# lunarlab-gatech/SLIDE_SLAM

Hardware: AMD Instinct MI355X
Metric: pose-graph updates/sec + ms/Gauss-Newton iter, 8-robot 10k-landmark graph (higher is better)
Workload: dtype f64

## Files before the change

### slide_slam_amd/csrc/solver_kernels.hip

```cpp
#include <hip/hip_runtime.h>
#include <algorithm>
#include <cstring>

#include "graph_dev.hpp"
#include "kernels.hpp"
#include "sl_math.hpp"

namespace sl {

struct BufPtrs { double* p[8]; };

__device__ inline void pose_retract12(const double* in12, const double* d6, int chart, double* out12) {
  to12(retract(from12(in12), d6, chart), out12);
}
__device__ inline void lm_retract(int type, const double* in, const double* d, int chart, double* out) {
  if (type == VT_POINT) {
    out[0] = in[0] + d[0]; out[1] = in[1] + d[1]; out[2] = in[2] + d[2];
  } else if (type == VT_CUBE) {
    pose_retract12(in, d, chart, out);
    out[12] = in[12] + d[6]; out[13] = in[13] + d[7]; out[14] = in[14] + d[8];
  } else {
    out[3] = in[3] + d[0]; out[4] = in[4] + d[1]; out[5] = in[5] + d[2];
    out[0] = in[0] + d[3]; out[1] = in[1] + d[4]; out[2] = in[2] + d[5];
    out[6] = in[6] + d[6];
// ... 928 lines not shown
void launch_gather_args(void* stage, const void* segs, int nseg, hipStream_t s) {
  GatherArgs A{};
  std::memcpy(A.seg, segs, (size_t)nseg * sizeof(ScatterSeg));
  if (nseg > 0) hipLaunchKernelGGL(k_gather_args, dim3(nseg, 4), dim3(256), 0, s, static_cast<unsigned char*>(stage), A);
}
void launch_gather(void* stage, unsigned desc_off, int nseg, hipStream_t s) {
  if (nseg > 0) hipLaunchKernelGGL(k_gather, dim3(nseg, 4), dim3(256), 0, s, static_cast<unsigned char*>(stage), desc_off);
}
void launch_scatter(const void* stage, unsigned desc_off, int nseg, hipStream_t s) {
  if (nseg > 0) hipLaunchKernelGGL(k_scatter, dim3(nseg, 8), dim3(256), 0, s, static_cast<const unsigned char*>(stage), desc_off);
}

__device__ __forceinline__ void k_pad_rhs_body(const GraphDev& G, int bid) {
  const int n = 6 * G.P, NT = G.T * NB;
  const long long t = (long long)bid * 256 + threadIdx.x;
  if (t < NT) {
    const int c = (int)t;
    G.S[(size_t)c * G.ld + NT + (size_t)G.nbr * NB] = c < G.col0 ? G.yv[c] : ((c < n) ? -G.pose_g[c] : 0.0);
    return;
  }
  const long long u = t - NT;
  const int npad = NT - n;
  if (u >= (long long)npad * NT) return;
  const int r = n + (int)(u / NT), c = (int)(u % NT);
  if (c > r || c < G.col0) return;
  if (G.first && c < G.first[G.T - 1] * NB) return;
  G.S[(size_t)c * G.ld + r] = (c == r) ? 1.0 : 0.0;
  if (G.save_S0) G.S0[(size_t)c * G.ld + r] = (c == r) ? 1.0 : 0.0;
}
__global__ __launch_bounds__(256) void k_pad_rhs(GraphDev G) { k_pad_rhs_body(G, blockIdx.x); }
__global__ __launch_bounds__(256) void k_pad_rhs_b(const GraphDev* __restrict__ Gs) {
  const GraphDev G = Gs[blockIdx.z];
  k_pad_rhs_body(G, blockIdx.x);
}

template <int MODE>
__device__ __forceinline__ void k_backsub_body(const GraphDev& G) {
  const int wave = threadIdx.x >> 6, lane = threadIdx.x & 63;
  if (MODE != 2) {
    const int t = blockIdx.x * 256 + threadIdx.x;
    if (t < 6 * G.P) G.pose_delta[t] = G.dp[t];
  }
  for (int l = blockIdx.x * 4 + wave; l < G.L; l += gridDim.x * 4) {
    const int D = lm_dim(G.lm_type[l]);
    double rhs[9];
#pragma unroll
    for (int k = 0; k < 9; ++k) rhs[k] = 0.0;
    if (MODE == 2) {
#pragma unroll
      for (int k = 0; k < 9; ++k) if (k < D) rhs[k] = G.lm_t[9 * (size_t)l + k];
    } else {
      for (int q = G.lm_ptr[l] + lane; q < G.lm_ptr[l + 1]; q += 64) {
        const int f = G.lm_fids[q];
        const double* E = G.ebuf + G.lf_eoff[f];
        const double* d = G.dp + 6 * (size_t)G.lf_pose[f];
        double dd[6];
#pragma unroll
        for (int a = 0; a < 6; ++a) dd[a] = d[a];
#pragma unroll
        for (int k = 0; k < 9; ++k) {
          if (k < D) {
            double s = 0.0;
#pragma unroll
            for (int a = 0; a < 6; ++a) s += E[a * D + k] * dd[a];
            rhs[k] += s;
          }
        }
      }
#pragma unroll
      for (int k = 0; k < 9; ++k) {
#pragma unroll
        for (int m = 32; m >= 1; m >>= 1) rhs[k] += __shfl_xor(rhs[k], m);
      }
    }
    if (MODE == 1) {
      if (lane == 0) {
#pragma unroll
        for (int k = 0; k < 9; ++k) G.lm_t[9 * (size_t)l + k] = rhs[k];
      }
      continue;
    }
#pragma unroll
    for (int k = 0; k < 9; ++k) if (k < D) rhs[k] += G.lm_g[9 * (size_t)l + k];
    if (lane < D) {
      const double* Hi = G.lm_Hinv + 81 * (size_t)l + lane * D;
      double s = 0.0;
#pragma unroll
      for (int c = 0; c < 9; ++c) if (c < D) s += Hi[c] * rhs[c];
      G.lm_delta[9 * (size_t)l + lane] = -s;
    }
  }
}
template <int MODE>
__global__ __launch_bounds__(256) void k_backsub(GraphDev G) { k_backsub_body<MODE>(G); }
template <int MODE>
__global__ __launch_bounds__(256) void k_backsub_b(const GraphDev* __restrict__ Gs) { k_backsub_body<MODE>(Gs[blockIdx.z]); }

__device__ __forceinline__ void k_shared_pack_body(const GraphDev& G, int what, double* __restrict__ buf) {
  const int w = what == 0 ? 54 : (what == 1 ? 9 : 15);
  const int t = blockIdx.x * blockDim.x + threadIdx.x;
  const int sidx = t / w, k = t - sidx * w;
  if (sidx >= G.n_slots) return;
  const int l = G.sh_lid[sidx];
  const bool live = l >= 0 && (what != 2 || G.sh_owner[sidx]);
  const double* src = what == 0 ? G.lm_Hacc + 54 * (size_t)(l < 0 ? 0 : l) : (what == 1 ? G.lm_t + 9 * (size_t)(l < 0 ? 0 : l) : G.lm_val + 15 * (size_t)(l < 0 ? 0 : l));
  buf[t] = live ? src[k] : 0.0;
}
__global__ void k_shared_pack(GraphDev G, int what, double* __restrict__ buf) { k_shared_pack_body(G, what, buf); }
__global__ void k_shared_unpack(GraphDev G, int what, const double* __restrict__ buf) {
  const int w = what == 0 ? 54 : (what == 1 ? 9 : 15);
  const int t = blockIdx.x * blockDim.x + threadIdx.x;
  const int sidx = t / w, k = t - sidx * w;
  if (sidx >= G.n_slots) return;
  const int l = G.sh_lid[sidx];
  if (l < 0) return;
  double* dst = what == 0 ? G.lm_Hacc + 54 * (size_t)l : (what == 1 ? G.lm_t + 9 * (size_t)l : G.lm_val + 15 * (size_t)l);
  const int nv = what == 2 ? (G.lm_type[l] == VT_POINT ? 3 : (G.lm_type[l] == VT_CUBE ? 15 : 7)) : w;
  if (k < nv) dst[k] = buf[t];
}

__global__ __launch_bounds__(256) void k_border_clear_b(const GraphDev* __restrict__ Gs) {
  const GraphDev G = Gs[blockIdx.z];
  if (!G.arrow || G.nbr <= 0) return;
  const long long nrow = (long long)G.nbr * NB, ncol = (long long)G.T * NB;
  const long long nb = (long long)(G.nbr + 1) * NB * G.nbr * NB;
  if (G.seg_tab) {
    const int* st = G.seg_tab;
    const int nseg = st[0], ntile = G.nbr * G.T;
    for (int tile = blockIdx.x; tile < ntile; tile += gridDim.x) {
      const int t = tile % G.nbr, c = tile / G.nbr;
      bool on = false;
      for (int q = 0; q < nseg; ++q) on = on || (st[1 + nseg + q * (G.nbr + 1) + t] <= c && c < st[1 + q]);
      if (!on) continue;
      double* base = G.S + (size_t)c * NB * G.ld + (size_t)(G.T + t) * NB;
      for (int e = threadIdx.x; e < NB * NB; e += 256) base[(size_t)(e >> 6) * G.ld + (e & 63)] = 0.0;
    }
    (void)nb;
    return;
  }
  for (long long t = (long long)blockIdx.x * 256 + threadIdx.x; t < nrow * ncol; t += (long long)gridDim.x * 256)
    G.S[(size_t)(t / nrow) * G.ld + (size_t)G.T * NB + (size_t)(t % nrow)] = 0.0;
}
__global__ __launch_bounds__(256) void k_border_fill_b(const GraphDev* __restrict__ Gs) {
  const GraphDev G = Gs[blockIdx.z];
  if (!G.arrow || G.nbr <= 0) return;
  const int sidx = blockIdx.x * 4 + (threadIdx.x >> 6), lane = threadIdx.x & 63;
  if (sidx >= G.n_slots) return;
  const int l = G.sh_lid[sidx];
  if (l < 0) return;
  const int o = G.lm_bord[l];
  if (o < 0) return;
  const int D = lm_dim(G.lm_type[l]);
  const int a = lane / D, k = lane - a * D;
  if (lane < 6 * D) {
    for (int q = G.lm_ptr[l]; q < G.lm_ptr[l + 1]; ++q) {
      const int f = G.lm_fids[q];
      const double e = G.ebuf[G.lf_eoff[f] + a * D + k];
      double* dst = G.S + (size_t)(6 * G.lf_pose[f] + a) * G.ld + (size_t)G.T * NB + o + k;
      *dst += e;
    }
  }
  const double* acc = G.lm_Hacc + 54 * (size_t)l;
  if (lane < D * (D + 1) / 2) {
    int r = 0;
    while ((r + 1) * (r + 2) / 2 <= lane) ++r;
    const int c = lane - r * (r + 1) / 2;
    G.bord0[(size_t)(o + c) * G.ldb + o + r] = acc[lane];
  }
  if (lane < D) G.bord0[(size_t)(o + lane) * G.ldb + (size_t)G.nbr * NB] = -acc[45 + lane];
}
__global__ __launch_bounds__(256) void k_sep_extract_b(const GraphDev* __restrict__ Gs, int max_sep) {
  const GraphDev G = Gs[blockIdx.z];
  if (!G.arrow || !G.pose_sep || G.nsep <= 0) return;
  __shared__ int s_q;
  if (threadIdx.x == 0) s_q = -1;
  __syncthreads();
  for (int p = threadIdx.x; p < G.P; p += 256)
    if (G.pose_sep[p] == 6 * (int)blockIdx.x) s_q = p;
  __syncthreads();
  const int q = s_q;
  if (q < 0) return;
  (void)max_sep;
  const int tid = threadIdx.x, oq = G.pose_sep[q], NT = G.T * NB;
  const size_t ld = G.ld, ldb = G.ldb;
  const size_t brow = (size_t)G.T * NB;
  const int nb_rows = G.nbr * NB;
  const int r_end = G.prof ? min(NT, (G.prof[(6 * q + 5) / NB] + 1) * NB) : NT;
  const int n_strip = r_end - 6 * q;
  const int part = blockIdx.y;
  for (int e = tid; part == 0 && e < 6 * n_strip; e += 256) {
    const int a = e / n_strip, r = 6 * q + e % n_strip, c = 6 * q + a;
    if (r < c) continue;
    double* src = G.S + (size_t)c * ld + r;
    const double v = *src;
    const int pr = r / 6;
    if (pr < G.P) {
      const int orr = G.pose_sep[pr];
      if (orr >= 0) G.bord0[(size_t)(oq + a) * ldb + orr + (r - 6 * pr)] = v;
      else G.S[(size_t)r * ld + brow + oq + a] = v;
    }
    *src = (r == c) ? 1.0 : 0.0;
  }
  for (int e = tid; part == 1 && e < 6 * nb_rows; e += 256) {
    const int a = e / nb_rows, b = e % nb_rows;
    double* src = G.S + (size_t)(6 * q + a) * ld + brow + b;
    const double v = *src;
    double* dst = G.bord0 + (size_t)(oq + a) * ldb + b;
    if (v != 0.0) { *dst = v; *src = 0.0; }
    else if (b >= G.nsep * NB && *dst != 0.0) *dst = 0.0;
  }
  if (part == 0 && tid < 6) {
    double* src = G.S + (size_t)(6 * q + tid) * ld + brow + (size_t)G.nbr * NB;
    G.bord0[(size_t)(oq + tid) * ldb + (size_t)G.nbr * NB] = *src;
    *src = 0.0;
  }
  if (part == 0 && blockIdx.x == 0)
    for (int p = G.nsep_dim + tid; p < G.nsep * NB; p += 256) G.bord0[(size_t)p * ldb + p] = 1.0;
  const int c_beg = G.first ? G.first[(6 * q) / NB] * NB : 0;
  for (int e = tid; part == 2 && e < 6 * (6 * q - c_beg); e += 256) {
    const int a = e % 6, c = c_beg + e / 6, r = 6 * q + a;
    const int pc = c / 6;
    if (pc >= G.P || G.pose_sep[pc] >= 0) continue;
    double* src = G.S + (size_t)c * ld + r;
    G.S[(size_t)c * ld + brow + oq + a] = *src;
    *src = 0.0;
  }
}
__global__ __launch_bounds__(256) void k_sep_pose_scatter_b(const GraphDev* __restrict__ Gs, BufPtrs X) {
  const GraphDev G = Gs[blockIdx.z];
  if (!G.arrow || !G.pose_sep || G.nsep <= 0) return;
  const int t = blockIdx.x * 256 + threadIdx.x;
  if (t >= 6 * G.P) return;
  const int o = G.pose_sep[t / 6];
  if (o >= 0) G.dp[t] = X.p[blockIdx.z][o + t % 6];
}
__global__ __launch_bounds__(256) void k_border_fill_lam_b(const GraphDev* __restrict__ Gs) {
  const GraphDev G = Gs[blockIdx.z];
  if (!G.arrow || !G.gh_bord || G.nbr <= 0) return;
  const int t = blockIdx.x * 256 + threadIdx.x;
  const int q = t / 36, e = t - 36 * q;
  if (q >= G.n_ghost) return;
  const int o = G.gh_bord[q];
  if (o < 0) return;
  const int k = e / 6, a = e - 6 * k;
  G.S[(size_t)(6 * G.gh_pose[q] + a) * G.ld + (size_t)G.T * NB + o + k] = G.gh_J[36 * (size_t)q + 6 * k + a];
  if (G.gh_first[q] && a == 0) {
    G.bord0[(size_t)(o + k) * G.ldb + o + k] = -1.0;
    G.bord0[(size_t)(o + k) * G.ldb + (size_t)G.nbr * NB] = -G.gh_r[6 * (size_t)q + k];
  }
}
__device__ __forceinline__ size_t sep_packed_addr(int row, int col, int Ts, int hTa, int hTL) {
  const int tj = col / NB, cc = col - tj * NB, hb = hTL - hTa;
  const size_t off = (size_t)(NB * NB) * ((size_t)tj * (Ts + 1) - (size_t)tj * (tj - 1) / 2 - (size_t)hb * min(tj, hTa));
  const int height = Ts + 1 - tj - (tj < hTa ? hb : 0);
  int r = row - tj * NB;
  if (tj < hTa && row >= hTL * NB) r -= hb * NB;
  return off + (size_t)cc * ((size_t)height * NB) + (size_t)r;
}
__device__ __forceinline__ bool sep_packed_hole(int row, int col, int hTa, int hTL) { return col < hTa * NB && row >= hTa * NB && row < hTL * NB; }
__device__ __forceinline__ double* sep_slot(const SepLayout& Y, int vr, int vc, bool packed) {
  const int Tt = Y.Ts + Y.nl;
  if (packed) return Y.packed + sep_packed_addr(vr, vc, Tt, Y.hTa, Y.hTL);
  if (vc < Y.Ts * NB) return Y.sys + (size_t)vc * ((size_t)(Tt + 1) * NB) + vr;
  return Y.bord + (size_t)(vc - Y.Ts * NB) * ((size_t)(Y.nl + 1) * NB) + (vr - Y.Ts * NB);
}
struct SepGatherArgs {
  int n, packed;
  SepLayout Y;
  const double* bord[8]; int ldb[8]; int nbr[8]; const int* map[8];
  const int* tmask;
  unsigned robot_mask;
  int split_col; unsigned mask_b; double* sys2; int ld2; double* bord2;
};
constexpr int SEP_GATHER_COLS = 8;
__global__ __launch_bounds__(256) void k_sep_gather(SepGatherArgs A) {
  const SepLayout& Y = A.Y;
  const int vr = blockIdx.x * 256 + threadIdx.x;
  const int NL = Y.Ts * NB, NT = (Y.Ts + Y.nl) * NB;
  if (vr > NT) return;
  const bool rhs = vr == NT;
  const int gr = rhs ? 0 : (vr < NL ? (vr < Y.ms ? vr : -1) : (vr - NL < Y.lam ? Y.ms + vr - NL : -1));
  const unsigned rmask = A.tmask ? (rhs ? ~0u : (unsigned)A.tmask[vr / NB]) : ~0u;
  int lrow[8];
#pragma unroll
  for (int r = 0; r < 8; ++r) {
    lrow[r] = -1;
    if (r < A.n && gr >= 0 && ((rmask >> r) & 1u) && ((A.robot_mask >> r) & 1u)) lrow[r] = rhs ? A.nbr[r] * NB : A.map[r][gr];
  }
#pragma unroll 2
  for (int vc = blockIdx.y * SEP_GATHER_COLS; vc < (int)(blockIdx.y + 1) * SEP_GATHER_COLS && vc < NT; ++vc) {
    if (!rhs && vr < vc) continue;
    if (sep_packed_hole(vr, vc, Y.hTa, Y.hTL)) continue;
    const int gc = vc < NL ? (vc < Y.ms ? vc : -1) : (vc - NL < Y.lam ? Y.ms + vc - NL : -1);
    double s = 0.0, s2 = 0.0;
    if (gc < 0 || gr < 0) {
      s = (vr == vc && vc < NL) ? 1.0 : 0.0;
    } else if (vr == vc && ((vc >= Y.gap[0] && vc < Y.gap[1]) || (vc >= Y.gap[2] && vc < Y.gap[3]))) {
      s = A.packed ? 0.0 : 1.0;
    } else {
      const unsigned cand = (A.tmask ? (unsigned)A.tmask[vc / NB] & rmask : ~0u) & A.robot_mask;
      double v[8];
#pragma unroll
      for (int r = 0; r < 8; ++r) {
        v[r] = 0.0;
        if (r < A.n && ((cand >> r) & 1u) && lrow[r] >= 0) {
          const int lc = A.map[r][gc];
          const int lr = lrow[r];
          if (lc >= 0) v[r] = A.bord[r][(size_t)min(lr, lc) * A.ldb[r] + max(lr, lc)];
        }
      }
      if (A.split_col >= 0 && vc >= A.split_col) {
        double va[8], vb[8];
#pragma unroll
        for (int r = 0; r < 8; ++r) { const bool b = (A.mask_b >> r) & 1u; va[r] = b ? 0.0 : v[r]; vb[r] = b ? v[r] : 0.0; }
        s = ((va[0] + va[1]) + (va[2] + va[3])) + ((va[4] + va[5]) + (va[6] + va[7]));
        s2 = ((vb[0] + vb[1]) + (vb[2] + vb[3])) + ((vb[4] + vb[5]) + (vb[6] + vb[7]));
      } else {
        s = ((v[0] + v[1]) + (v[2] + v[3])) + ((v[4] + v[5]) + (v[6] + v[7]));
      }
    }
    *sep_slot(Y, vr, vc, A.packed != 0) = s;
    if (A.split_col >= 0 && vc >= A.split_col) {
      if (vc < NL) A.sys2[(size_t)(vc - A.split_col) * A.ld2 + (vr - A.split_col)] = s2;
      else A.bord2[(size_t)(vc - NL) * ((size_t)(Y.nl + 1) * NB) + (vr - NL)] = s2;
    }
  }
}
__global__ __launch_bounds__(256) void k_sep_unpack(SepLayout Y, int c0, int c1, int to_packed) {
  const int vr = blockIdx.x * 256 + threadIdx.x, vc = c0 * NB + blockIdx.y;
  const int NT = (Y.Ts + Y.nl) * NB;
  if (vr > NT || vc >= NT || vc >= c1 * NB || vr < vc / NB * NB) return;
  if (sep_packed_hole(vr, vc, Y.hTa, Y.hTL)) return;
  if (to_packed) { *sep_slot(Y, vr, vc, true) = *sep_slot(Y, vr, vc, false); return; }
  double v = *sep_slot(Y, vr, vc, true);
  if (vr == vc && ((vc >= Y.gap[0] && vc < Y.gap[1]) || (vc >= Y.gap[2] && vc < Y.gap[3]))) v = 1.0;
  *sep_slot(Y, vr, vc, false) = v;
}
__global__ __launch_bounds__(256) void k_lam_prepare(const double* __restrict__ bord, int nl, int lam, double* __restrict__ out) {
  const int r = blockIdx.x * 256 + threadIdx.x, c = blockIdx.y;
  const int NT = nl * NB, ld = (nl + 1) * NB;
  if (r > NT || c >= NT) return;
  const bool rhs = r == NT;
  if (!rhs && r < c) return;
  double v;
  if (c < lam && (rhs || r < lam)) v = -bord[(size_t)c * ld + r];
  else v = (r == c) ? 1.0 : 0.0;
  out[(size_t)c * ld + r] = v;
}
struct SepScatterArgs { int n, m, ms; const double* xs; const double* xl; double* xloc[8]; const int* map[8]; };
__global__ __launch_bounds__(256) void k_sep_xloc(SepScatterArgs A) {
  const int g = blockIdx.x * 256 + threadIdx.x, r = blockIdx.y;
  if (g >= A.m || r >= A.n) return;
  const int lc = A.map[r][g];
  if (lc >= 0) A.xloc[r][lc] = g < A.ms ? A.xs[g] : A.xl[g - A.ms];
}
__global__ __launch_bounds__(256) void k_sep_lm_delta_b(const GraphDev* __restrict__ Gs, SepScatterArgs A, const int* __restrict__ sep_off) {
  const GraphDev G = Gs[blockIdx.z];
  const int t = blockIdx.x * 256 + threadIdx.x;
  const int sidx = t / 9, k = t - 9 * sidx;
  if (sidx >= G.n_slots) return;
  const int l = G.sh_lid[sidx];
  if (l < 0) return;
  if (k < lm_dim(G.lm_type[l])) G.lm_delta[9 * (size_t)l + k] = A.xs[sep_off[sidx] + k];
}
__global__ void k_ghost_exchange(GraphDev G, int what, double* __restrict__ buf) {
  const int t = blockIdx.x * blockDim.x + threadIdx.x;
  if (t >= 12 * G.n_gslots) return;
  if (what == 0) {
    const int p = G.gslot_pose[t / 12];
    buf[t] = p >= 0 ? G.pose_est[12 * (size_t)p + t % 12] : 0.0;
  } else {
    G.ghost_val[t] = buf[t];
  }
}

struct GhostBufs { double* p[8]; };
__global__ void k_ghost_exchange_b(const GraphDev* __restrict__ Gs, int what, GhostBufs B) {
  const GraphDev G = Gs[blockIdx.z];
  double* buf = B.p[blockIdx.z];
  const int t = blockIdx.x * blockDim.x + threadIdx.x;
  if (t >= 12 * G.n_gslots) return;
  if (what == 0) {
    const int p = G.gslot_pose[t / 12];
    buf[t] = p >= 0 ? G.pose_est[12 * (size_t)p + t % 12] : 0.0;
  } else {
    G.ghost_val[t] = buf[t];
  }
}
__global__ void k_ghost_refresh_local(const GraphDev* __restrict__ Gs, int n) {
  const GraphDev G = Gs[blockIdx.z];
  const int t = blockIdx.x * blockDim.x + threadIdx.x;
  if (t >= 12 * G.n_gslots) return;
  double v = 0.0;
  for (int q = 0; q < n; ++q) {
    const int p = Gs[q].gslot_pose[t / 12];
    v += p >= 0 ? Gs[q].pose_est[12 * (size_t)p + t % 12] : 0.0;
  }
  G.ghost_val[t] = v;
}
void launch_ghost_refresh_local(const GraphDev* d, int n, int n_gslots, hipStream_t s) {
  if (n_gslots <= 0 || n <= 0) return;
  hipLaunchKernelGGL(k_ghost_refresh_local, dim3((12 * n_gslots + 127) / 128, 1, n), dim3(128), 0, s, d, n);
}
void launch_ghost_exchange_batched(const GraphDev* d, int n, int n_gslots, int what, double* const* bufs, hipStream_t s) {
  if (n_gslots <= 0 || n <= 0) return;
  GhostBufs B{};
  for (int i = 0; i < n; ++i) B.p[i] = bufs[i];
  hipLaunchKernelGGL(k_ghost_exchange_b, dim3((12 * n_gslots + 127) / 128, 1, n), dim3(128), 0, s, d, what, B);
}

__device__ __forceinline__ void k_estimate_body(const GraphDev& G) {
  const int t = blockIdx.x * blockDim.x + threadIdx.x;
  if (t < G.P) {
    pose_retract12(G.pose_val + 12 * (size_t)t, G.pose_delta + 6 * (size_t)t, G.chart, G.pose_est + 12 * (size_t)t);
  } else if (t < G.P + G.L) {
    const int l = t - G.P;
    lm_retract(G.lm_type[l], G.lm_val + 15 * (size_t)l, G.lm_delta + 9 * (size_t)l, G.chart, G.lm_est + 15 * (size_t)l);
  }
}
__global__ void k_estimate(GraphDev G) { k_estimate_body(G); }
__global__ void k_estimate_predict(GraphDev G, int pose, double* __restrict__ out) {
  k_estimate_body(G);
  const int t = blockIdx.x * blockDim.x + threadIdx.x;
  int dirty = 0;
  if (t < G.P) {
    double mx = 0.0;
#pragma unroll
    for (int k = 0; k < 6; ++k) mx = fmax(mx, fabs(G.pose_delta[6 * (size_t)t + k]));
    if (mx >= G.relin_thr) dirty = mark_dirty_pose(G, t);
  } else if (t < G.P + G.L) {
    const int l = t - G.P;
    const int d = lm_dim(G.lm_type[l]);
    double mx = 0.0;
    for (int k = 0; k < d; ++k) mx = fmax(mx, fabs(G.lm_delta[9 * (size_t)l + k]));
    if (mx >= G.relin_thr) dirty = mark_dirty_lm(G, l);
  }
  if (__ballot(dirty > 0)) {
#pragma unroll
    for (int off = 32; off > 0; off >>= 1) dirty = max(dirty, __shfl_xor(dirty, off));
    if ((threadIdx.x & 63) == 0 && dirty > 0) atomicMax(&G.status[5], dirty);
  }
  if (out) {
    __shared__ int s_last;
    __threadfence();
    __syncthreads();
    if (threadIdx.x == 0) {
      int* cnt = reinterpret_cast<int*>(out + 16);
      const int a = atomicAdd(cnt, 1);
      s_last = (a == (int)gridDim.x - 1) ? 1 : 0;
      if (s_last) *cnt = 0;
    }
    __syncthreads();
    if (s_last) {
      __threadfence();
      const int tt = threadIdx.x;
      if (tt < 8) {
        reinterpret_cast<int*>(out)[tt] = __hip_atomic_load(&G.status[tt], __ATOMIC_RELAXED, __HIP_MEMORY_SCOPE_AGENT);
        G.status[tt] = 0;
      } else if (tt < 20) {
        out[4 + (tt - 8)] = pose >= 0 ? __hip_atomic_load(&G.pose_est[12 * (size_t)pose + (tt - 8)], __ATOMIC_RELAXED, __HIP_MEMORY_SCOPE_AGENT) : 0.0;
      }
    }
  }
}
__global__ void k_final_pack(GraphDev G, int pose, double* __restrict__ out) {
  const int t = threadIdx.x;
  if (t < 8) {
    reinterpret_cast<int*>(out)[t] = G.status[t];
    G.status[t] = 0;
  } else if (t < 20) {
    out[4 + (t - 8)] = pose >= 0 ? G.pose_est[12 * (size_t)pose + (t - 8)] : 0.0;
  }
// ... 37 lines not shown
  const int npf = G.n_prior + G.n_between + G.n_ghost;
  if (G.n_lf > 0) {
    const int nb0 = npf > 0 ? (int)blocks_for(npf, 256) : 0;
    hipLaunchKernelGGL(k_lin_lf, dim3(nb0 + blocks_for(G.n_lf, 256) + blocks_for(32LL * G.n_lf, 256)), dim3(256), 0, s, G, nb0, (int)blocks_for(G.n_lf, 256));
  } else if (npf > 0) {
    hipLaunchKernelGGL(k_lin_pose_factors, dim3(blocks_for(npf, 128)), dim3(128), 0, s, G);
  }
}
void launch_landmark(const GraphDev& G, int mode, hipStream_t s) {
  if (G.L == 0) return;
  if (mode == 0) hipLaunchKernelGGL(k_landmark<0>, dim3(blocks_for(G.L, 4)), dim3(256), 0, s, G);
  else if (mode == 1) hipLaunchKernelGGL(k_landmark<1>, dim3(blocks_for(G.L, 4)), dim3(256), 0, s, G);
  else hipLaunchKernelGGL(k_landmark<2>, dim3(blocks_for(G.L, 4)), dim3(256), 0, s, G);
}
void launch_pose(const GraphDev& G, hipStream_t s) {
  if (G.P > 0) hipLaunchKernelGGL(k_pose, dim3(blocks_for(G.P, 4)), dim3(256), 0, s, G);
}
void launch_schur(const GraphDev& G, hipStream_t s) {
  if (G.P == 0) return;
  static const int env_split = getenv("SLIDE_SCHUR_SPLIT") ? atoi(getenv("SLIDE_SCHUR_SPLIT")) : 0;
  const int split = env_split > 0 ? env_split : (G.schur_split > 0 ? G.schur_split : 2);
  const long long NT = (long long)G.T * NB;
  const long long tot = NT + (NT - 6LL * G.P) * NT;
  const int p_first = G.col0 > 5 ? std::min((G.col0 - 5 + 5) / 6, G.P) : 0;
  hipLaunchKernelGGL(k_schur, dim3((unsigned)(G.P - p_first) + (unsigned)blocks_for(tot, 256), split > 0 ? split : 1), dim3(256),
                     (size_t)((G.L + 7) / 8 * 8) * sizeof(short) + (size_t)((G.P + 31) / 32 + 1) * sizeof(unsigned), s, G, p_first);
}
void launch_backsub(const GraphDev& G, int mode, hipStream_t s) {
  if (G.P + G.L == 0) return;
  const int nb = std::max(blocks_for(G.L, 4), blocks_for(6 * G.P, 256));
  if (mode == 0) hipLaunchKernelGGL(k_backsub<0>, dim3(nb), dim3(256), 0, s, G);
  else if (mode == 1) hipLaunchKernelGGL(k_backsub<1>, dim3(nb), dim3(256), 0, s, G);
  else hipLaunchKernelGGL(k_backsub<2>, dim3(nb), dim3(256), 0, s, G);
}
__global__ void k_shared_unpack_b(const GraphDev* __restrict__ Gs, int what, BufPtrs B) {
  const GraphDev G = Gs[blockIdx.z];
  const int w = what == 0 ? 54 : (what == 1 ? 9 : 15);
  const int t = blockIdx.x * blockDim.x + threadIdx.x;
  const int sidx = t / w, k = t - sidx * w;
  if (sidx >= G.n_slots) return;
  const int l = G.sh_lid[sidx];
  if (l < 0) return;
  double* dst = what == 0 ? G.lm_Hacc + 54 * (size_t)l : (what == 1 ? G.lm_t + 9 * (size_t)l : G.lm_val + 15 * (size_t)l);
  const int nv = what == 2 ? (G.lm_type[l] == VT_POINT ? 3 : (G.lm_type[l] == VT_CUBE ? 15 : 7)) : w;
  if (k < nv) dst[k] = B.p[blockIdx.z][t];
}
void launch_phase3_batched(const GraphDev* d, const GraphDev* h, int n, double* const* bufs, hipStream_t s) {
  int L = 0, P = 0, slots = 0;
  long long pad = 0;
  for (int i = 0; i < n; ++i) {
    L = std::max(L, h[i].L); P = std::max(P, h[i].P); slots = std::max(slots, h[i].n_slots);
    const long long NT = (long long)h[i].T * NB;
    pad = std::max(pad, NT + (NT - 6LL * h[i].P) * NT);
  }
  BufPtrs B{};
  for (int i = 0; i < n; ++i) B.p[i] = bufs[i];
  if (slots > 0) hipLaunchKernelGGL(k_shared_unpack_b, dim3(blocks_for(54LL * slots, 128), 1, n), dim3(128), 0, s, d, 0, B);
  if (L > 0) hipLaunchKernelGGL(k_landmark_b<2>, dim3(blocks_for(L, 4), 1, n), dim3(256), 0, s, d);
  if (P > 0) {
    hipLaunchKernelGGL(k_pose_b, dim3(blocks_for(P, 4), 1, n), dim3(256), 0, s, d);
    static const int env_split = getenv("SLIDE_SCHUR_SPLIT") ? atoi(getenv("SLIDE_SCHUR_SPLIT")) : 0;
    int split = 1;
    for (int i = 0; i < n; ++i) split = std::max(split, h[i].schur_split > 0 ? h[i].schur_split : 2);
    if (env_split > 0) split = env_split;
    hipLaunchKernelGGL(k_schur_b, dim3(P, split > 0 ? split : 1, n), dim3(256),
                       (size_t)((L + 7) / 8 * 8) * sizeof(short) + (size_t)((P + 31) / 32 + 1) * sizeof(unsigned), s, d);
    hipLaunchKernelGGL(k_pad_rhs_b, dim3(blocks_for(pad, 256), 1, n), dim3(256), 0, s, d);
  }
}
void launch_phase3_arrow_batched(const GraphDev* d, const GraphDev* h, int n, hipStream_t s) {
  int L = 0, P = 0;
  long long pad = 0;
  for (int i = 0; i < n; ++i) {
    L = std::max(L, h[i].L); P = std::max(P, h[i].P);
    const long long NT = (long long)h[i].T * NB;
    pad = std::max(pad, NT + (NT - 6LL * h[i].P) * NT);
  }
  if (L > 0) hipLaunchKernelGGL(k_landmark_b<3>, dim3(blocks_for(L, 4), 1, n), dim3(256), 0, s, d);
  if (P > 0) {
    hipLaunchKernelGGL(k_pose_b, dim3(blocks_for(P, 4), 1, n), dim3(256), 0, s, d);
    int split = 1;
    bool listed = true;
    for (int i = 0; i < n; ++i) { split = std::max(split, h[i].schur_split > 0 ? h[i].schur_split : 2); listed = listed && h[i].sp_idx != nullptr; }
    const size_t lds = (size_t)((L + 7) / 8 * 8) * sizeof(short) + (size_t)((P + 31) / 32 + 1) * sizeof(unsigned);
    static const int schur_xcd = getenv("SLIDE_SCHUR_XCD") ? atoi(getenv("SLIDE_SCHUR_XCD")) : 0;
    if (listed) hipLaunchKernelGGL(k_schur_lb, dim3(P, split > 0 ? split : 1, n), dim3(256), lds, s, d, schur_xcd);
    else hipLaunchKernelGGL(k_schur_b, dim3(P, split > 0 ? split : 1, n), dim3(256), lds, s, d);
    hipLaunchKernelGGL(k_pad_rhs_b, dim3(blocks_for(pad, 256), 1, n), dim3(256), 0, s, d);
  }
  launch_border_assemble_batched(d, h, n, s);
}
__global__ void k_shared_pack_b(const GraphDev* __restrict__ Gs, int what, BufPtrs B) { k_shared_pack_body(Gs[blockIdx.z], what, B.p[blockIdx.z]); }
void launch_phase0_batched(const GraphDev* d, const GraphDev* h, int n, double* const* bufs, hipStream_t s, bool pack) {
  int L = 0, P = 0, slots = 0, npf = 0;
  long long nlf = 0;
  for (int i = 0; i < n; ++i) {
    L = std::max(L, h[i].L); P = std::max(P, h[i].P); slots = std::max(slots, h[i].n_slots);
    npf = std::max(npf, h[i].n_prior + h[i].n_between + h[i].n_ghost);
    nlf = std::max<long long>(nlf, h[i].n_lf);
  }
  BufPtrs B{};
  for (int i = 0; i < n; ++i) B.p[i] = bufs[i];
  if (P + L > 0) hipLaunchKernelGGL(k_relin_b, dim3(blocks_for(P + L, 256), 1, n), dim3(256), 0, s, d);
  if (nlf > 0) {
    const int nb0 = npf > 0 ? (int)blocks_for(npf, 256) : 0;
    hipLaunchKernelGGL(k_lin_lf_b, dim3(nb0 + blocks_for(nlf, 256) + blocks_for(32LL * nlf, 256), 1, n), dim3(256), 0, s, d, nb0, (int)blocks_for(nlf, 256));
  } else if (npf > 0) {
    hipLaunchKernelGGL(k_lin_pose_factors_b, dim3(blocks_for(npf, 128), 1, n), dim3(128), 0, s, d);
  }
  if (L > 0 && pack) hipLaunchKernelGGL(k_landmark_b<1>, dim3(blocks_for(L, 4), 1, n), dim3(256), 0, s, d);
  if (slots > 0 && pack) hipLaunchKernelGGL(k_shared_pack_b, dim3(blocks_for(54LL * slots, 128), 1, n), dim3(128), 0, s, d, 0, B);
}
void launch_phase4_batched(const GraphDev* d, const GraphDev* h, int n, double* const* bufs, hipStream_t s) {
  int L = 0, P = 0, slots = 0;
  for (int i = 0; i < n; ++i) { L = std::max(L, h[i].L); P = std::max(P, h[i].P); slots = std::max(slots, h[i].n_slots); }
  BufPtrs B{};
  for (int i = 0; i < n; ++i) B.p[i] = bufs[i];
  if (P + L > 0) hipLaunchKernelGGL(k_backsub_b<1>, dim3(std::max(blocks_for(L, 4), blocks_for(6 * P, 256)), 1, n), dim3(256), 0, s, d);
  if (slots > 0) hipLaunchKernelGGL(k_shared_pack_b, dim3(blocks_for(9LL * slots, 128), 1, n), dim3(128), 0, s, d, 1, B);
}
void launch_phase2_batched(const GraphDev* d, const GraphDev* h, int n, double* const* bufs, hipStream_t s) {
  int L = 0, P = 0, slots = 0;
  for (int i = 0; i < n; ++i) { L = std::max(L, h[i].L); P = std::max(P, h[i].P); slots = std::max(slots, h[i].n_slots); }
  BufPtrs B{};
  for (int i = 0; i < n; ++i) B.p[i] = bufs[i];
  if (slots > 0) hipLaunchKernelGGL(k_shared_unpack_b, dim3(blocks_for(9LL * slots, 128), 1, n), dim3(128), 0, s, d, 1, B);
  if (P + L > 0) {
    hipLaunchKernelGGL(k_backsub_b<2>, dim3(std::max(blocks_for(L, 4), blocks_for(6 * P, 256)), 1, n), dim3(256), 0, s, d);
    hipLaunchKernelGGL(k_estimate_b, dim3(blocks_for(P + L, 256), 1, n), dim3(256), 0, s, d);
  }
}
void launch_shared_pack(const GraphDev& G, int what, double* buf, hipStream_t s) {
  if (G.n_slots > 0) hipLaunchKernelGGL(k_shared_pack, dim3(blocks_for(54LL * G.n_slots, 128)), dim3(128), 0, s, G, what, buf);
}
void launch_shared_unpack(const GraphDev& G, int what, const double* buf, hipStream_t s) {
  if (G.n_slots > 0) hipLaunchKernelGGL(k_shared_unpack, dim3(blocks_for(54LL * G.n_slots, 128)), dim3(128), 0, s, G, what, buf);
}
void launch_ghost_exchange(const GraphDev& G, int what, double* buf, hipStream_t s) {
  if (G.n_gslots > 0) hipLaunchKernelGGL(k_ghost_exchange, dim3(blocks_for(12LL * G.n_gslots, 128)), dim3(128), 0, s, G, what, buf);
}
void launch_estimate(const GraphDev& G, hipStream_t s) {
  if (G.P + G.L == 0) return;
  hipLaunchKernelGGL(k_estimate, dim3(blocks_for(G.P + G.L, 256)), dim3(256), 0, s, G);
}
void launch_estimate_predict(const GraphDev& G, hipStream_t s, int pose, double* out17) {
  if (G.P + G.L == 0) return;
  hipLaunchKernelGGL(k_estimate_predict, dim3(blocks_for(G.P + G.L, 256)), dim3(256), 0, s, G, pose, out17);
}
void launch_final_pack(const GraphDev& G, int pose, double* out16, hipStream_t s) {
  hipLaunchKernelGGL(k_final_pack, dim3(1), dim3(64), 0, s, G, pose, out16);
}

void launch_sep_extract_batched(const GraphDev* d, const GraphDev* h, int n, const int* n_sep_poses, hipStream_t s) {
  int mx = 0;
  for (int i = 0; i < n; ++i) mx = std::max(mx, (h[i].arrow && h[i].pose_sep) ? n_sep_poses[i] : 0);
  if (mx > 0) hipLaunchKernelGGL(k_sep_extract_b, dim3(mx, 3, n), dim3(256), 0, s, d, mx);
}
void launch_sep_pose_scatter_batched(const GraphDev* d, const GraphDev* h, int n, double* const* xloc, hipStream_t s) {
  int P = 0;
  bool any = false;
  for (int i = 0; i < n; ++i) { P = std::max(P, h[i].P); any = any || (h[i].arrow && h[i].pose_sep && h[i].nsep > 0); }
  if (!any || P == 0) return;
  BufPtrs X{};
  for (int i = 0; i < n; ++i) X.p[i] = xloc[i];
  hipLaunchKernelGGL(k_sep_pose_scatter_b, dim3(blocks_for(6LL * P, 256), 1, n), dim3(256), 0, s, d, X);
}
void launch_border_assemble_batched(const GraphDev* d, const GraphDev* h, int n, hipStream_t s) {
  int slots = 0;
  long long work = 0;
  for (int i = 0; i < n; ++i) {
    slots = std::max(slots, h[i].n_slots);
    work = std::max(work, (long long)h[i].nbr * NB * h[i].T * NB);
  }
  if (work <= 0 || slots <= 0) return;
  hipLaunchKernelGGL(k_border_clear_b, dim3((unsigned)std::min<long long>((work + 255) / 256, 4096), 1, n), dim3(256), 0, s, d);
  hipLaunchKernelGGL(k_border_fill_b, dim3((slots + 3) / 4, 1, n), dim3(256), 0, s, d);
  int ngh = 0;
  for (int i = 0; i < n; ++i) ngh = std::max(ngh, h[i].gh_bord ? h[i].n_ghost : 0);
  if (ngh > 0) hipLaunchKernelGGL(k_border_fill_lam_b, dim3((36 * ngh + 255) / 256, 1, n), dim3(256), 0, s, d);
}
void launch_sep_unpack(const SepLayout& Y, hipStream_t s, int c0, int c1, bool to_packed) {
  const int NT = (Y.Ts + Y.nl) * NB;
  if (c1 < 0) c1 = Y.Ts + Y.nl;
  if (NT > 0 && c1 > c0) hipLaunchKernelGGL(k_sep_unpack, dim3((NT + 1 + 255) / 256, (c1 - c0) * NB), dim3(256), 0, s, Y, c0, c1, to_packed ? 1 : 0);
}
__global__ __launch_bounds__(256) void k_sep_top_add(SepLayout Y, int c0, const double* __restrict__ sys2, int ld2, const double* __restrict__ bord2) {
  const int vr = blockIdx.x * 256 + threadIdx.x, vc = c0 * NB + blockIdx.y;
  const int NL = Y.Ts * NB, NT = (Y.Ts + Y.nl) * NB;
  if (vr > NT || vc >= NT || vr < vc / NB * NB) return;
  double* dst = sep_slot(Y, vr, vc, false);
  if (vc < NL) *dst += sys2[(size_t)(vc - c0 * NB) * ld2 + (vr - c0 * NB)];
  else *dst += bord2[(size_t)(vc - NL) * ((size_t)(Y.nl + 1) * NB) + (vr - NL)];
}
void launch_sep_top_add(const SepLayout& Y, int c0, const double* sys2, int ld2, const double* bord2, hipStream_t s) {
  const int NT = (Y.Ts + Y.nl) * NB;
  const int ncol = NT - c0 * NB;
  if (ncol > 0) hipLaunchKernelGGL(k_sep_top_add, dim3((NT + 1 + 255) / 256, ncol), dim3(256), 0, s, Y, c0, sys2, ld2, bord2);
}
void launch_sep_gather(const GraphDev* h, int n, const int* const* maps, const SepLayout& Y, bool packed, hipStream_t s, const int* tmask,
                       int split_col, unsigned mask_b, double* sys2, int ld2, double* bord2) {
  SepGatherArgs A{};
  A.n = n; A.Y = Y; A.packed = packed ? 1 : 0; A.tmask = tmask;
  A.robot_mask = ~0u; A.split_col = split_col; A.mask_b = mask_b; A.sys2 = sys2; A.ld2 = ld2; A.bord2 = bord2;
  for (int i = 0; i < n; ++i) { A.bord[i] = h[i].bord; A.ldb[i] = h[i].ldb; A.nbr[i] = h[i].nbr; A.map[i] = maps[i]; }
  const int NT = (Y.Ts + Y.nl) * NB;
  if (NT > 0) hipLaunchKernelGGL(k_sep_gather, dim3((NT + 1 + 255) / 256, (NT + SEP_GATHER_COLS - 1) / SEP_GATHER_COLS), dim3(256), 0, s, A);
}
void launch_lam_prepare(const double* bord, int nl, int lam, double* out, hipStream_t s) {
  if (nl > 0) hipLaunchKernelGGL(k_lam_prepare, dim3((nl * NB + 1 + 255) / 256, nl * NB), dim3(256), 0, s, bord, nl, lam, out);
}
void launch_sep_xloc(int n, const int* const* maps, int ms, int lam, const double* xs, const double* xl, double* const* xloc, hipStream_t s) {
  SepScatterArgs A{};
  A.n = n; A.m = ms + lam; A.ms = ms; A.xs = xs; A.xl = xl;
  for (int i = 0; i < n; ++i) { A.xloc[i] = xloc[i]; A.map[i] = maps[i]; }
  if (A.m > 0) hipLaunchKernelGGL(k_sep_xloc, dim3((A.m + 255) / 256, n), dim3(256), 0, s, A);
}
void launch_arrow_finish_batched(const GraphDev* d, const GraphDev* h, int n, const double* xs, const int* sep_off, hipStream_t s) {
  int L = 0, P = 0, slots = 0;
  for (int i = 0; i < n; ++i) { L = std::max(L, h[i].L); P = std::max(P, h[i].P); slots = std::max(slots, h[i].n_slots); }
  if (P + L == 0) return;
  hipLaunchKernelGGL(k_backsub_b<0>, dim3(std::max(blocks_for(L, 4), blocks_for(6 * P, 256)), 1, n), dim3(256), 0, s, d);
  SepScatterArgs A{};
  A.n = n; A.xs = xs;
  if (slots > 0) hipLaunchKernelGGL(k_sep_lm_delta_b, dim3(blocks_for(9LL * slots, 256), 1, n), dim3(256), 0, s, d, A, sep_off);
  hipLaunchKernelGGL(k_estimate_b, dim3(blocks_for(P + L, 256), 1, n), dim3(256), 0, s, d);
}

}
```

Before: 3749.

## Restructure border fill, separator extract, and separator gather kernels for coalescing

Three kernels change. The border fill now batches landmark factor metadata across lanes with shuffles and overwrites first-touch entries instead of accumulating into them. The separator extract splits border copying across more blocks with vectorized double2 accesses and batches strided loads in groups of four. The separator gather becomes a 64x16 tile kernel that stages robot index maps and transposed border tiles in shared memory, replacing per-element scattered min/max lookups with coalesced reads. These changes aim to cut uncoalesced global traffic and load latency in separator assembly, at the cost of more complex indexing, extra barriers, and reliance on the assumption that first writes can replace accumulation.

Result: faster. 3878, median of 6 (+3.5%).

```diff
diff --git a/slide_slam_amd/csrc/solver_kernels.hip b/slide_slam_amd/csrc/solver_kernels.hip
--- a/slide_slam_amd/csrc/solver_kernels.hip
+++ b/slide_slam_amd/csrc/solver_kernels.hip
@@ -1104,14 +1104,7 @@
   if (o < 0) return;
   const int D = lm_dim(G.lm_type[l]);
   const int a = lane / D, k = lane - a * D;
-  if (lane < 6 * D) {
-    for (int q = G.lm_ptr[l]; q < G.lm_ptr[l + 1]; ++q) {
-      const int f = G.lm_fids[q];
-      const double e = G.ebuf[G.lf_eoff[f] + a * D + k];
-      double* dst = G.S + (size_t)(6 * G.lf_pose[f] + a) * G.ld + (size_t)G.T * NB + o + k;
-      *dst += e;
-    }
-  }
+  const int p0 = G.lm_ptr[l], p1 = G.lm_ptr[l + 1];
   const double* acc = G.lm_Hacc + 54 * (size_t)l;
   if (lane < D * (D + 1) / 2) {
     int r = 0;
@@ -1120,6 +1113,41 @@
     G.bord0[(size_t)(o + c) * G.ldb + o + r] = acc[lane];
   }
   if (lane < D) G.bord0[(size_t)(o + lane) * G.ldb + (size_t)G.nbr * NB] = -acc[45 + lane];
+  const bool live = lane < 6 * D;
+  double* const col0 = G.S + (size_t)a * G.ld + (size_t)G.T * NB + o + k;
+  for (int base = p0; base < p1; base += 64) {
+    const int nq = min(64, p1 - base);
+    int pose = -1, eoff = 0;
+    if (lane < nq) {
+      const int f = G.lm_fids[base + lane];
+      pose = G.lf_pose[f];
+      eoff = G.lf_eoff[f];
+    }
+    bool again = base > p0;
+    for (int j = 0; j < nq; ++j) {
+      const int pj = __shfl(pose, j);
+      again = again || (j < lane && pj == pose);
+    }
+    const unsigned long long again_mask = __ballot(again);
+    for (int j0 = 0; j0 < nq; j0 += 8) {
+      double e[8];
+      int pj[8];
+#pragma unroll
+      for (int u = 0; u < 8; ++u) {
+        const int ej = __shfl(eoff, j0 + u);
+        pj[u] = __shfl(pose, j0 + u);
+        e[u] = 0.0;
+        if (live && j0 + u < nq) e[u] = G.ebuf[ej + lane];
+      }
+#pragma unroll
+      for (int u = 0; u < 8; ++u) {
+        if (!live || j0 + u >= nq) continue;
+        double* dst = col0 + (size_t)6 * pj[u] * G.ld;
+        if ((again_mask >> (j0 + u)) & 1ull) *dst += e[u];
+        else *dst = 0.0 + e[u];
+      }
+    }
+  }
 }
 __global__ __launch_bounds__(256) void k_sep_extract_b(const GraphDev* __restrict__ Gs, int max_sep) {
   const GraphDev G = Gs[blockIdx.z];
@@ -1133,33 +1161,55 @@
   const int q = s_q;
   if (q < 0) return;
   (void)max_sep;
-  const int tid = threadIdx.x, oq = G.pose_sep[q], NT = G.T * NB;
+  const int tid = threadIdx.x, oq = 6 * (int)blockIdx.x, NT = G.T * NB;
   const size_t ld = G.ld, ldb = G.ldb;
   const size_t brow = (size_t)G.T * NB;
   const int nb_rows = G.nbr * NB;
+  const int part = blockIdx.y;
+  if (part >= 2) {
+    const int n4 = nb_rows / 4, e = (part - 2) * 256 + tid;
+    if (e >= 6 * n4) return;
+    const int a = e / n4, b0 = 4 * (e - a * n4);
+    double* src = G.S + (size_t)(6 * q + a) * ld + brow + b0;
+    double* dst = G.bord0 + (size_t)(oq + a) * ldb + b0;
+    const double2 v01 = *reinterpret_cast<const double2*>(src), v23 = *reinterpret_cast<const double2*>(src + 2);
+    const double2 d01 = *reinterpret_cast<const double2*>(dst), d23 = *reinterpret_cast<const double2*>(dst + 2);
+    const double v[4] = {v01.x, v01.y, v23.x, v23.y}, d[4] = {d01.x, d01.y, d23.x, d23.y};
+#pragma unroll
+    for (int k = 0; k < 4; ++k) {
+      if (v[k] != 0.0) { dst[k] = v[k]; src[k] = 0.0; }
+      else if (b0 + k >= G.nsep * NB && d[k] != 0.0) dst[k] = 0.0;
+    }
+    return;
+  }
   const int r_end = G.prof ? min(NT, (G.prof[(6 * q + 5) / NB] + 1) * NB) : NT;
   const int n_strip = r_end - 6 * q;
-  const int part = blockIdx.y;
-  for (int e = tid; part == 0 && e < 6 * n_strip; e += 256) {
-    const int a = e / n_strip, r = 6 * q + e % n_strip, c = 6 * q + a;
-    if (r < c) continue;
-    double* src = G.S + (size_t)c * ld + r;
-    const double v = *src;
-    const int pr = r / 6;
-    if (pr < G.P) {
-      const int orr = G.pose_sep[pr];
-      if (orr >= 0) G.bord0[(size_t)(oq + a) * ldb + orr + (r - 6 * pr)] = v;
-      else G.S[(size_t)r * ld + brow + oq + a] = v;
-    }
-    *src = (r == c) ? 1.0 : 0.0;
-  }
-  for (int e = tid; part == 1 && e < 6 * nb_rows; e += 256) {
-    const int a = e / nb_rows, b = e % nb_rows;
-    double* src = G.S + (size_t)(6 * q + a) * ld + brow + b;
-    const double v = *src;
-    double* dst = G.bord0 + (size_t)(oq + a) * ldb + b;
-    if (v != 0.0) { *dst = v; *src = 0.0; }
-    else if (b >= G.nsep * NB && *dst != 0.0) *dst = 0.0;
+  for (int e0 = tid; part == 0 && e0 < 6 * n_strip; e0 += 4 * 256) {
+    double v[4];
+    int orr[4];
+#pragma unroll
+    for (int u = 0; u < 4; ++u) {
+      const int e = e0 + 256 * u;
+      v[u] = 0.0; orr[u] = -1;
+      if (e >= 6 * n_strip) continue;
+      const int a = e / n_strip, r = 6 * q + e % n_strip, c = 6 * q + a;
+      if (r < c) continue;
+      v[u] = G.S[(size_t)c * ld + r];
+      if (r / 6 < G.P) orr[u] = G.pose_sep[r / 6];
+    }
+#pragma unroll
+    for (int u = 0; u < 4; ++u) {
+      const int e = e0 + 256 * u;
+      if (e >= 6 * n_strip) continue;
+      const int a = e / n_strip, r = 6 * q + e % n_strip, c = 6 * q + a;
+      if (r < c) continue;
+      const int pr = r / 6;
+      if (pr < G.P) {
+        if (orr[u] >= 0) G.bord0[(size_t)(oq + a) * ldb + orr[u] + (r - 6 * pr)] = v[u];
+        else G.S[(size_t)r * ld + brow + oq + a] = v[u];
+      }
+      G.S[(size_t)c * ld + r] = (r == c) ? 1.0 : 0.0;
+    }
   }
   if (part == 0 && tid < 6) {
     double* src = G.S + (size_t)(6 * q + tid) * ld + brow + (size_t)G.nbr * NB;
@@ -1169,13 +1219,28 @@
   if (part == 0 && blockIdx.x == 0)
     for (int p = G.nsep_dim + tid; p < G.nsep * NB; p += 256) G.bord0[(size_t)p * ldb + p] = 1.0;
   const int c_beg = G.first ? G.first[(6 * q) / NB] * NB : 0;
-  for (int e = tid; part == 2 && e < 6 * (6 * q - c_beg); e += 256) {
-    const int a = e % 6, c = c_beg + e / 6, r = 6 * q + a;
-    const int pc = c / 6;
-    if (pc >= G.P || G.pose_sep[pc] >= 0) continue;
-    double* src = G.S + (size_t)c * ld + r;
-    G.S[(size_t)c * ld + brow + oq + a] = *src;
-    *src = 0.0;
+  const int n_row = 6 * (6 * q - c_beg);
+  for (int e0 = tid; part == 1 && e0 < n_row; e0 += 4 * 256) {
+    double v[4];
+    int oc[4];
+#pragma unroll
+    for (int u = 0; u < 4; ++u) {
+      const int e = e0 + 256 * u;
+      v[u] = 0.0; oc[u] = 0;
+      if (e >= n_row) continue;
+      const int a = e % 6, c = c_beg + e / 6;
+      if (c / 6 >= G.P) continue;
+      oc[u] = G.pose_sep[c / 6];
+      v[u] = G.S[(size_t)c * ld + 6 * q + a];
+    }
+#pragma unroll
+    for (int u = 0; u < 4; ++u) {
+      const int e = e0 + 256 * u;
+      if (e >= n_row || oc[u] >= 0) continue;
+      const int a = e % 6, c = c_beg + e / 6;
+      G.S[(size_t)c * ld + brow + oq + a] = v[u];
+      G.S[(size_t)c * ld + 6 * q + a] = 0.0;
+    }
   }
 }
 __global__ __launch_bounds__(256) void k_sep_pose_scatter_b(const GraphDev* __restrict__ Gs, BufPtrs X) {
@@ -1224,52 +1289,107 @@
   unsigned robot_mask;
   int split_col; unsigned mask_b; double* sys2; int ld2; double* bord2;
 };
-constexpr int SEP_GATHER_COLS = 8;
+constexpr int SEP_GATHER_COLS = 16;
 __global__ __launch_bounds__(256) void k_sep_gather(SepGatherArgs A) {
   const SepLayout& Y = A.Y;
-  const int vr = blockIdx.x * 256 + threadIdx.x;
-  const int NL = Y.Ts * NB, NT = (Y.Ts + Y.nl) * NB;
-  if (vr > NT) return;
-  const bool rhs = vr == NT;
-  const int gr = rhs ? 0 : (vr < NL ? (vr < Y.ms ? vr : -1) : (vr - NL < Y.lam ? Y.ms + vr - NL : -1));
-  const unsigned rmask = A.tmask ? (rhs ? ~0u : (unsigned)A.tmask[vr / NB]) : ~0u;
-  int lrow[8];
-#pragma unroll
-  for (int r = 0; r < 8; ++r) {
-    lrow[r] = -1;
-    if (r < A.n && gr >= 0 && ((rmask >> r) & 1u) && ((A.robot_mask >> r) & 1u)) lrow[r] = rhs ? A.nbr[r] * NB : A.map[r][gr];
-  }
-#pragma unroll 2
-  for (int vc = blockIdx.y * SEP_GATHER_COLS; vc < (int)(blockIdx.y + 1) * SEP_GATHER_COLS && vc < NT; ++vc) {
+  const int tr = blockIdx.x, c0 = blockIdx.y * SEP_GATHER_COLS, tc = c0 / NB;
+  const int Tt = Y.Ts + Y.nl, NL = Y.Ts * NB, NT = Tt * NB;
+  if (tr < tc) return;
+  if (tc < Y.hTa && tr >= Y.hTa && tr < Y.hTL) return;
+  const bool rhs = tr == Tt;
+  const int tid = threadIdx.x;
+  __shared__ int s_l[8][NB + SEP_GATHER_COLS];
+  __shared__ double s_t[2][SEP_GATHER_COLS][NB + 1];
+  unsigned cand = A.robot_mask & ((1u << A.n) - 1u);
+  if (A.tmask) cand &= (unsigned)A.tmask[tc] & (rhs ? ~0u : (unsigned)A.tmask[tr]);
+  auto coord = [&](int v) { return v < NL ? (v < Y.ms ? v : -1) : (v - NL < Y.lam ? Y.ms + v - NL : -1); };
+  if (cand != 0) {
+    if (tid < NB + SEP_GATHER_COLS) {
+      const bool row = tid < NB;
+      const int g = row ? (rhs ? (tid == 0 ? 0 : -1) : coord(tr * NB + tid)) : coord(c0 + tid - NB);
+#pragma unroll
+      for (int r = 0; r < 8; ++r) {
+        int l = -1;
+        if (((cand >> r) & 1u) && g >= 0) l = (row && rhs) ? A.nbr[r] * NB : A.map[r][g];
+        s_l[r][tid] = l;
+      }
+    }
+    __syncthreads();
+  }
+  const int i = tid & (NB - 1), j0 = (tid >> 6) * 4;
+  const int jb = tid & (SEP_GATHER_COLS - 1), i0 = (tid >> 4) * 4;
+  const int vr = rhs ? NT : tr * NB + i;
+  const bool row_live = !rhs || i == 0;
+  double ha[2][4], hb[2][4];
+#pragma unroll
+  for (int p = 0; p < 4; ++p) {
+    double w[2][4], v[2][4];
+#pragma unroll
+    for (int rr = 0; rr < 2; ++rr)
+#pragma unroll
+      for (int jj = 0; jj < 4; ++jj) v[rr][jj] = 0.0;
+    if (((cand >> (2 * p)) & 3u) != 0) {
+#pragma unroll
+      for (int rr = 0; rr < 2; ++rr) {
+        const int r = 2 * p + rr;
+        const int lc = s_l[r][NB + jb];
+#pragma unroll
+        for (int ii = 0; ii < 4; ++ii) {
+          const int lr = s_l[r][i0 + ii];
+          w[rr][ii] = 0.0;
+          if (lc >= 0 && lr >= 0 && lr < lc && tr * NB + i0 + ii >= c0 + jb) w[rr][ii] = A.bord[r][(size_t)lr * A.ldb[r] + lc];
+        }
+      }
+#pragma unroll
+      for (int rr = 0; rr < 2; ++rr) {
+        const int r = 2 * p + rr;
+        const int lr = s_l[r][i];
+#pragma unroll
+        for (int jj = 0; jj < 4; ++jj) {
+          const int lc = s_l[r][NB + j0 + jj];
+          if (lc >= 0 && lr >= lc && (rhs || vr >= c0 + j0 + jj)) v[rr][jj] = A.bord[r][(size_t)lc * A.ldb[r] + lr];
+        }
+      }
+#pragma unroll
+      for (int rr = 0; rr < 2; ++rr)
+#pragma unroll
+        for (int ii = 0; ii < 4; ++ii) s_t[rr][jb][i0 + ii] = w[rr][ii];
+      __syncthreads();
+#pragma unroll
+      for (int rr = 0; rr < 2; ++rr) {
+        const int r = 2 * p + rr;
+        const int lr = s_l[r][i];
+#pragma unroll
+        for (int jj = 0; jj < 4; ++jj) {
+          const int lc = s_l[r][NB + j0 + jj];
+          if (lc >= 0 && lr >= 0 && lr < lc) v[rr][jj] = s_t[rr][j0 + jj][i];
+        }
+      }
+      __syncthreads();
+    }
+#pragma unroll
+    for (int jj = 0; jj < 4; ++jj) {
+      const bool split = A.split_col >= 0 && c0 + j0 + jj >= A.split_col;
+      const bool b0 = split && ((A.mask_b >> (2 * p)) & 1u), b1 = split && ((A.mask_b >> (2 * p + 1)) & 1u);
+      const double qa = (b0 ? 0.0 : v[0][jj]) + (b1 ? 0.0 : v[1][jj]), qb = (b0 ? v[0][jj] : 0.0) + (b1 ? v[1][jj] : 0.0);
+      if (p & 1) { ha[p / 2][jj] += qa; hb[p / 2][jj] += qb; }
+      else { ha[p / 2][jj] = qa; hb[p / 2][jj] = qb; }
+    }
+  }
+  if (!row_live) return;
+  const int gr = rhs ? 0 : coord(vr);
+#pragma unroll
+  for (int jj = 0; jj < 4; ++jj) {
+    const int vc = c0 + j0 + jj;
     if (!rhs && vr < vc) continue;
-    if (sep_packed_hole(vr, vc, Y.hTa, Y.hTL)) continue;
-    const int gc = vc < NL ? (vc < Y.ms ? vc : -1) : (vc - NL < Y.lam ? Y.ms + vc - NL : -1);
-    double s = 0.0, s2 = 0.0;
+    const int gc = coord(vc);
+    double s = ha[0][jj] + ha[1][jj], s2 = hb[0][jj] + hb[1][jj];
     if (gc < 0 || gr < 0) {
       s = (vr == vc && vc < NL) ? 1.0 : 0.0;
+      s2 = 0.0;
     } else if (vr == vc && ((vc >= Y.gap[0] && vc < Y.gap[1]) || (vc >= Y.gap[2] && vc < Y.gap[3]))) {
       s = A.packed ? 0.0 : 1.0;
-    } else {
-      const unsigned cand = (A.tmask ? (unsigned)A.tmask[vc / NB] & rmask : ~0u) & A.robot_mask;
-      double v[8];
-#pragma unroll
-      for (int r = 0; r < 8; ++r) {
-        v[r] = 0.0;
-        if (r < A.n && ((cand >> r) & 1u) && lrow[r] >= 0) {
-          const int lc = A.map[r][gc];
-          const int lr = lrow[r];
-          if (lc >= 0) v[r] = A.bord[r][(size_t)min(lr, lc) * A.ldb[r] + max(lr, lc)];
-        }
-      }
-      if (A.split_col >= 0 && vc >= A.split_col) {
-        double va[8], vb[8];
-#pragma unroll
-        for (int r = 0; r < 8; ++r) { const bool b = (A.mask_b >> r) & 1u; va[r] = b ? 0.0 : v[r]; vb[r] = b ? v[r] : 0.0; }
-        s = ((va[0] + va[1]) + (va[2] + va[3])) + ((va[4] + va[5]) + (va[6] + va[7]));
-        s2 = ((vb[0] + vb[1]) + (vb[2] + vb[3])) + ((vb[4] + vb[5]) + (vb[6] + vb[7]));
-      } else {
-        s = ((v[0] + v[1]) + (v[2] + v[3])) + ((v[4] + v[5]) + (v[6] + v[7]));
-      }
+      s2 = 0.0;
     }
     *sep_slot(Y, vr, vc, A.packed != 0) = s;
     if (A.split_col >= 0 && vc >= A.split_col) {
@@ -1613,9 +1733,10 @@
 }
 
 void launch_sep_extract_batched(const GraphDev* d, const GraphDev* h, int n, const int* n_sep_poses, hipStream_t s) {
-  int mx = 0;
-  for (int i = 0; i < n; ++i) mx = std::max(mx, (h[i].arrow && h[i].pose_sep) ? n_sep_poses[i] : 0);
-  if (mx > 0) hipLaunchKernelGGL(k_sep_extract_b, dim3(mx, 3, n), dim3(256), 0, s, d, mx);
+  int mx = 0, nbr = 0;
+  for (int i = 0; i < n; ++i)
+    if (h[i].arrow && h[i].pose_sep && n_sep_poses[i] > 0) { mx = std::max(mx, n_sep_poses[i]); nbr = std::max(nbr, h[i].nbr); }
+  if (mx > 0) hipLaunchKernelGGL(k_sep_extract_b, dim3(mx, 2 + (6 * nbr * (NB / 4) + 255) / 256, n), dim3(256), 0, s, d, mx);
 }
 void launch_sep_pose_scatter_batched(const GraphDev* d, const GraphDev* h, int n, double* const* xloc, hipStream_t s) {
   int P = 0;
@@ -1665,7 +1786,8 @@
   A.robot_mask = ~0u; A.split_col = split_col; A.mask_b = mask_b; A.sys2 = sys2; A.ld2 = ld2; A.bord2 = bord2;
   for (int i = 0; i < n; ++i) { A.bord[i] = h[i].bord; A.ldb[i] = h[i].ldb; A.nbr[i] = h[i].nbr; A.map[i] = maps[i]; }
   const int NT = (Y.Ts + Y.nl) * NB;
-  if (NT > 0) hipLaunchKernelGGL(k_sep_gather, dim3((NT + 1 + 255) / 256, (NT + SEP_GATHER_COLS - 1) / SEP_GATHER_COLS), dim3(256), 0, s, A);
+  static_assert(NB % SEP_GATHER_COLS == 0 && SEP_GATHER_COLS == 16, "k_sep_gather: a strip lies in one tile column, four columns per thread");
+  if (NT > 0) hipLaunchKernelGGL(k_sep_gather, dim3(Y.Ts + Y.nl + 1, NT / SEP_GATHER_COLS), dim3(256), 0, s, A);
 }
 void launch_lam_prepare(const double* bord, int nl, int lam, double* out, hipStream_t s) {
   if (nl > 0) hipLaunchKernelGGL(k_lam_prepare, dim3((nl * NB + 1 + 255) / 256, nl * NB), dim3(256), 0, s, bord, nl, lam, out);
```
